# zkcrypto/bls12_381

Hardware: AMD Instinct MI355X
Metric: G1 MSM throughput (scalar-muls/sec) at 2^20 points (higher is better)
Workload: dtype u32 (14x28-bit limbs, 64-bit accumulators); 1 GPU; 2^20-point G1 MSM per MI355X, bases resident in HBM, scalars in HBM; one result per step; points_per_gpu=1048576, total_points=1048576, parallelism=shard1

## Files before the change

### bls12_381_amd/csrc/api_ctx.hip

```cpp
#define BLS_TU_NAME "api_ctx.hip"
#include "host.h"
#include "generators.hip.h"

__global__ void __launch_bounds__(256) k_fp_op(int op, const u32* __restrict__ a, const u32* __restrict__ b, u32* __restrict__ out, size_t n) {
  size_t i = (size_t)blockIdx.x * blockDim.x + threadIdx.x;
  if (i >= n) return;
  fe1 x = fe_from_ref(a + i * 12);
  fe1 y = b ? fe_from_ref(b + i * 12) : x;
  switch (op) {
    case 0: fe_to_ref(mul(x, y), out + i * 12); break;
    case 1: fe_to_ref(add(x, y), out + i * 12); break;
    case 2: fe_to_ref(sub(x, y), out + i * 12); break;
    case 3: fe_to_ref(sqr(x), out + i * 12); break;
    case 4: fe_to_ref(inv(x), out + i * 12); break;
    case 6: fe_to_ref(from_v16<2>(fe_inv_fermat_raw(to_v16(x))), out + i * 12); break;
    default: fe_to_ref(neg(x), out + i * 12); break;
  }
}
__global__ void __launch_bounds__(256) k_fp2_op(int op, const u32* __restrict__ a, const u32* __restrict__ b, u32* __restrict__ out, size_t n) {
  size_t i = (size_t)blockIdx.x * blockDim.x + threadIdx.x;
  if (i >= n) return;
  fe2_1 x = fe2_from_ref(a + i * 24);
  fe2_1 y = b ? fe2_from_ref(b + i * 24) : x;
  switch (op) {
// ... 145 lines not shown
  if (hipGetDeviceCount(&n) != hipSuccess || n <= 0) { g_err = "no HIP device"; return BLSGPU_ERR_NODEV; }
  if (device < 0 || device >= n) return bad("blsgpu_create: device index out of range");
  HIPCHK(hipSetDevice(device));
  blsgpu_ctx* c = new blsgpu_ctx();
  c->device = device;
  c->diag = diag_read(MMLP_MAX_K, ITEM_CAP_MAX, FR_COLS_LOG_MAX);
  if (c->diag.pairing_layout < 0) { delete c; return bad("blsgpu_create: BLSGPU_PAIRING_LAYOUT must be one of auto, pair, quad, wide"); }
  c->force_slow_sort = c->diag.force_slow_sort; c->no_glv = c->diag.no_glv; c->pairing_layout = c->diag.pairing_layout;
  c->mmlp_k = c->diag.mmlp_k; c->mml_impl = c->diag.mml_impl; c->h2c_split = c->diag.h2c_split; c->fr_cols_want = c->diag.fr_cols_want; c->item_cap = c->diag.item_cap;
  int rc = ctx_init(c);
  if (rc != BLSGPU_OK) { blsgpu_destroy(c); return rc; }
  *out = c;
  return BLSGPU_OK;
}
extern "C" void blsgpu_destroy(blsgpu_ctx* c) {
  if (!c) return;
  hipSetDevice(c->device);
  hipDeviceSynchronize();
  if (c->d_status) hipFree(c->d_status);
  if (c->d_wide) hipFree(c->d_wide);
  DevBuf* bufs[] = {&c->result, &c->io_a, &c->io_b, &c->io_c, &c->io_d, &c->io_e, &c->io_f, &c->io_out, &c->flags_a, &c->flags_b, &c->mml_vals, &c->fr_tw[0], &c->fr_tw[1], &c->fr_tmp, &c->fr_ninv, &c->fr_cs[0], &c->fr_cs[1], &c->fb_table[0], &c->fb_table[1], &c->fb_stage, &c->mmlp_work, &c->mmlp_out, &c->gt_one, &c->ver, &c->fold_c, &c->fold_d, &c->fold_result, &c->h2c_uniform, &c->seg_wsum, &c->seg_rec, &c->frs_agg[0], &c->frs_agg[1], &c->frs_carry[0], &c->frs_carry[1], &c->frs_lane};
  for (auto b : bufs) b->release();
  for (auto& sl : c->slot) {
    DevBuf* sb[] = {&sl.ent, &sl.sorted, &sl.hist, &sl.offs, &sl.cursor, &sl.bsum, &sl.items, &sl.heavy, &sl.ctrl, &sl.glv,
                    &sl.buckets, &sl.lvlR[0], &sl.lvlR[1], &sl.lvlT, &sl.tsum[0], &sl.tsum[1], &sl.wacc[0], &sl.wacc[1], &sl.wsums, &sl.result};
    for (auto b : sb) b->release();
    hipEvent_t evs[] = {sl.ev_in, sl.ev_front, sl.ev_acc, sl.ev_tail, sl.ev_k0, sl.ev_k1, sl.ev_tree};
    for (auto e : evs) if (e) hipEventDestroy(e);
    for (auto& e : sl.ev_lvl) if (e) hipEventDestroy(e);
    hipStream_t sts[] = {sl.front, sl.tail, sl.tail2};
    for (auto q : sts) if (q) hipStreamDestroy(q);
  }
  for (auto& e : c->ev) if (e) hipEventDestroy(e);
  for (auto& e : c->ev_fr) if (e) hipEventDestroy(e);
  for (auto& e : c->ev_fr_cs) if (e) hipEventDestroy(e);
  for (auto& e : c->ev_fb) if (e) hipEventDestroy(e);
  if (c->ev_gt_one) hipEventDestroy(c->ev_gt_one);
  if (c->fold_stream) hipStreamDestroy(c->fold_stream);
  if (c->pin_stage) hipHostFree(c->pin_stage);
  for (auto e : c->pin_ev) if (e) hipEventDestroy(e);
  if (c->ev_ver) hipEventDestroy(c->ev_ver);
  for (auto q : c->ver_stream) if (q) hipStreamDestroy(q);
  for (auto e : c->ev_ver_side) if (e) hipEventDestroy(e);
  if (c->ver_table) blsgpu_g2_prepared_free(c->ver_table);
  for (auto& e : c->bcache) if (e.b) blsgpu_bases_free(e.b);
  c->ktimer.destroy();
  if (c->acc_stream) hipStreamDestroy(c->acc_stream);
// ... 166 lines not shown
```

### bls12_381_amd/csrc/api_msm.hip

```cpp
#define BLS_TU_NAME "api_msm.hip"
#include "host.h"
#include "abi_kernels.hip.h"
#include "mulbatch.hip.h"
#include "msm_seg.hip.h"
#include "gntt.hip.h"

static void bases_drop(blsgpu_bases* b) {
  if (b->rec) hipFree(b->rec);
  if (b->endo) hipFree(b->endo);
  if (b->table) hipFree(b->table);
  if (b->ev_ready) hipEventDestroy(b->ev_ready);
  delete b;
}
static int bases_make_endo(blsgpu_ctx* c, blsgpu_bases* b, bool trusted) {
  if (!b->n) { b->subgroup = 1; return BLSGPU_OK; }
  if (b->group == 2 && b->n > ((size_t)1 << 22)) { b->subgroup = trusted ? 1 : (c->assume_subgroup ? 2 : 3); return BLSGPU_OK; }
  if (trusted) b->subgroup = 1;
  else if (c->assume_subgroup) b->subgroup = 2;
  else {
    u32 nbad = 0;
    HIPCHK(hipMemsetAsync(c->d_status + 1, 0, 4, c->stream));
    if (b->group == 1) KLAUNCH(k_bases_subgroup_check<FpPolicy>, dim3(nblk(b->n, 128)), dim3(128), 0, c->stream, b->rec, b->n, c->d_status + 1);
    else KLAUNCH(k_bases_subgroup_check<Fp2Policy>, dim3(nblk(b->n, 128)), dim3(128), 0, c->stream, b->rec, b->n, c->d_status + 1);
    LAUNCHCHK();
// ... 189 lines not shown
    KLAUNCH(k_proj_export<F>, dim3(1), dim3(256), 0, st, c->result.as<u32>(), (u32*)d_out_wire, (size_t)1);
    LAUNCHCHK();
    return BLSGPU_OK;
  }
  const bool merged = bases->table != nullptr;
  const bool glv = GroupTag<F>::id == 1 && !merged && bases->endo && !c->no_glv && !c->force_slow_sort && 2 * n <= ((size_t)1 << 24);
  const bool gls = GroupTag<F>::id == 2 && !merged && bases->endo && !c->no_glv && !c->force_slow_sort && 4 * n <= ((size_t)1 << 24);
  const size_t ns = glv ? 2 * n : gls ? 4 * n : n;
  const int sbits = glv ? 128 : gls ? 64 : 256;
  const int cw = merged ? bases->table_c : (c->msm_c ? c->msm_c : pick_window(ns, sbits));
  const int nwin = (sbits + cw - 1) / cw;
  const int nseg = merged ? 1 : nwin;
  const u32 nbw = 1u << (cw - 1);
  const size_t nb = (size_t)nseg * nbw;
  const size_t total = (size_t)nwin * ns;
  if (total > 0xfffffff0ull) return bad("msm: n * windows exceeds 2^32 entries");
  const bool fast_sort = merged || ((ns <= ((size_t)1 << 24)) && cw <= 16 && cw >= 2 && !c->force_slow_sort);
  const int key_bits = cw - 1;
  const int coarse_bits = merged ? (key_bits > 7 ? key_bits - 7 : 0) : (key_bits < 8 ? key_bits : 8);
  const int fine_bits = key_bits - coarse_bits;
  const int ncoarse = 1 << coarse_bits;
  const int nc = nseg * ncoarse;
  if (fast_sort && nc > SORT_MAX_COUNTERS) return bad("msm: window configuration exceeds the sort's counter table");
  if (!fast_sort && nblk(nb, 1024) > 4096) return bad("msm: too many buckets for the fallback sort (use a window <= 16)");
  int bad_alloc = 0;
  blsgpu_ctx::Slot& sl = c->slot[c->next_slot];
  c->next_slot = (c->next_slot + 1) % NSLOT;
  const bool single = !c->pipelining;
  hipStream_t ft = single ? st : sl.front, tt = single ? st : sl.tail;
  if (sl.tail_pending) { HIPCHK(hipStreamWaitEvent(ft, sl.ev_tail, 0)); HIPCHK(hipStreamWaitEvent(st, sl.ev_tail, 0)); }
  bad_alloc |= sl.ent.reserve(total * 4);
  bad_alloc |= sl.sorted.reserve(total * 4);
  {
    size_t hb = (nb > 3 * (size_t)SORT_MAX_COUNTERS + 4 ? nb : 3 * (size_t)SORT_MAX_COUNTERS + 4) * 4;
    bool fresh = sl.hist.cap < hb;
    bad_alloc |= sl.hist.reserve(hb);
    if (fresh && !bad_alloc) HIPCHK(hipMemsetAsync(sl.hist.p, 0, sl.hist.cap, ft));
  }
  if (!fast_sort) bad_alloc |= sl.cursor.reserve(total * 4);
  const int sform = c->scalar_form;
  const bool plain_mont = sform == SCALAR_MONT && !glv && !gls;
  if (glv) bad_alloc |= sl.glv.reserve(ns * 16);
  if (gls) bad_alloc |= sl.glv.reserve(ns * 8);
  if (plain_mont) bad_alloc |= sl.glv.reserve(n * 32);
  bad_alloc |= sl.offs.reserve((nb + 1) * 4);
  bad_alloc |= sl.bsum.reserve(4096 * 4);
  u32 cap = 128;
  while (cap < ITEM_CAP_MAX && (size_t)cap * nbw < 4 * ns) cap *= 2;
  if (c->item_cap) cap = c->item_cap;
  const size_t max_items = total / cap + nb + 1;
  const size_t max_records = nb + max_items;
  {
    blsgpu_ctx::Slot* g = &sl;
    bad_alloc |= g->items.reserve(max_items * sizeof(ItemDesc));
    bad_alloc |= g->heavy.reserve(2 * nb * sizeof(uint4));
    bad_alloc |= g->ctrl.reserve((4 + 2 * ITEM_BINS) * 4);
    size_t lvl = (nb / 2 + 1) * PW * 4;
    bool grow = g->buckets.cap < max_records * PW * 4 || g->lvlR[0].cap < lvl || g->lvlT.cap < 2 * lvl || g->wacc[0].cap < (size_t)nwin * 32 * PW * 4 || g->wsums.cap < (size_t)nwin * PW * 4;
    if (grow) { HIPCHK(hipStreamSynchronize(g->tail)); HIPCHK(hipStreamSynchronize(g->tail2)); HIPCHK(hipStreamSynchronize(st)); }
    bad_alloc |= g->buckets.reserve(max_records * PW * 4);
    bad_alloc |= g->lvlR[0].reserve(lvl); bad_alloc |= g->lvlR[1].reserve(lvl); bad_alloc |= g->lvlT.reserve(2 * lvl);
    bad_alloc |= g->tsum[0].reserve(lvl); bad_alloc |= g->tsum[1].reserve(lvl);
    bad_alloc |= g->wacc[0].reserve((size_t)nwin * 32 * PW * 4); bad_alloc |= g->wacc[1].reserve((size_t)nwin * 32 * PW * 4);
    bad_alloc |= g->wsums.reserve((size_t)nwin * PW * 4);
    bad_alloc |= g->result.reserve(PW * 4);
  }
  if (bad_alloc) { g_err = "hipMalloc(msm scratch) failed"; return BLSGPU_ERR_HIP; }
  const bool prof = c->profiling;
  auto mark = [&](int i) { if (prof) hipEventRecord(c->ev[i], ft); };
  if (ft != st) { HIPCHK(hipEventRecord(sl.ev_in, st)); HIPCHK(hipStreamWaitEvent(ft, sl.ev_in, 0)); }

  mark(0);
  if (plain_mont) {
    KLAUNCH(k_scalars_from_mont, dim3(nblk(n, 256)), dim3(256), 0, ft, (const u32*)d_scalars, sl.glv.as<u32>(), (int)n, c->status_word);
    LAUNCHCHK();
    d_scalars = sl.glv.p;
  }
  if (fast_sort) {
    u32* ghist = sl.hist.as<u32>();
    u32* gbase = ghist + SORT_MAX_COUNTERS;
    u32* gcur = gbase + SORT_MAX_COUNTERS + 1;
    if (sl.hist_dirty) { HIPCHK(hipMemsetAsync(ghist, 0, (size_t)SORT_MAX_COUNTERS * 4, ft)); sl.hist_dirty = false; }
    const unsigned tiles = nblk(ns, SORT_TILE);
    const u32* sort_in = (const u32*)d_scalars;
    if (glv) {
      KLAUNCH(k_glv_decompose, dim3(nblk(n, 256)), dim3(256), 0, ft, (const u32*)d_scalars, sl.glv.as<u32>(), (int)n, c->status_word, sform);
      sort_in = sl.glv.as<u32>();
      KLAUNCH(k_sort_hist<4>, dim3(tiles), dim3(SORT_THREADS), (size_t)nc * 4, ft, sort_in, ghist, (int)ns, cw, nwin, fine_bits, ncoarse, 0, c->status_word);
    } else if (gls) {
      KLAUNCH(k_gls_decompose, dim3(nblk(n, 256)), dim3(256), 0, ft, (const u32*)d_scalars, sl.glv.as<u32>(), (int)n, c->status_word, sform);
      sort_in = sl.glv.as<u32>();
      KLAUNCH(k_sort_hist<2>, dim3(tiles), dim3(SORT_THREADS), (size_t)nc * 4, ft, sort_in, ghist, (int)ns, cw, nwin, fine_bits, ncoarse, 0, c->status_word);
    } else {
      KLAUNCH(k_sort_hist<8>, dim3(tiles), dim3(SORT_THREADS), (size_t)nc * 4, ft, sort_in, ghist, (int)ns, cw, nwin, fine_bits, ncoarse, merged ? 1 : 0, c->status_word);
    }
    LAUNCHCHK();
    mark(1);
    KLAUNCH(k_sort_scan, dim3(1), dim3(1024), 0, ft, ghist, gbase, gcur, nc, sl.ctrl.as<u32>(), 4 + 2 * ITEM_BINS);
    LAUNCHCHK();
    mark(2);
    if (glv)
      KLAUNCH(k_sort_scatter<4>, dim3(tiles), dim3(SORT_THREADS), (size_t)nc * 8, ft, sort_in, gbase, gcur, sl.ent.as<u32>(), (int)ns, cw, nwin, fine_bits, ncoarse, 0, (u32)0);
    else if (gls)
      KLAUNCH(k_sort_scatter<2>, dim3(tiles), dim3(SORT_THREADS), (size_t)nc * 8, ft, sort_in, gbase, gcur, sl.ent.as<u32>(), (int)ns, cw, nwin, fine_bits, ncoarse, 0, (u32)0);
    else
      KLAUNCH(k_sort_scatter<8>, dim3(tiles), dim3(SORT_THREADS), (size_t)nc * 8, ft, sort_in, gbase, gcur, sl.ent.as<u32>(), (int)ns, cw, nwin,
                         fine_bits, ncoarse, merged ? 1 : 0, (u32)bases->n);
    KLAUNCH(k_sort_fine, dim3(nc), dim3(256), 0, ft, sl.ent.as<u32>(), gbase, sl.sorted.as<u32>(), sl.offs.as<u32>(), fine_bits, nc);
    LAUNCHCHK();
    mark(3);
  } else {
    sl.hist_dirty = true;
    HIPCHK(hipMemsetAsync(sl.hist.p, 0, nb * 4, ft));
    HIPCHK(hipMemsetAsync(sl.ctrl.p, 0, (4 + 2 * ITEM_BINS) * 4, ft));
    KLAUNCH(k_msm_digits, dim3(nblk(n, 256)), dim3(256), 0, ft, (const u32*)d_scalars, sl.ent.as<u32>(), sl.cursor.as<u32>(), sl.hist.as<u32>(), (int)n, cw, nwin, c->status_word);
    LAUNCHCHK();
    mark(1);
    unsigned sb = nblk(nb, 1024);
    KLAUNCH(k_scan_block_sums, dim3(sb), dim3(256), 0, ft, sl.hist.as<u32>(), sl.bsum.as<u32>(), (int)nb);
    KLAUNCH(k_scan_top, dim3(1), dim3(1024), 0, ft, sl.bsum.as<u32>(), (int)sb);
    KLAUNCH(k_scan_apply, dim3(sb), dim3(256), 0, ft, sl.hist.as<u32>(), sl.bsum.as<u32>(), sl.offs.as<u32>(), (int)nb);
    LAUNCHCHK();
    mark(2);
    KLAUNCH(k_msm_scatter, dim3(nblk(total, 256)), dim3(256), 0, ft, sl.ent.as<u32>(), sl.cursor.as<u32>(), sl.offs.as<u32>(), sl.sorted.as<u32>(),
                       (int)n, total);
    LAUNCHCHK();
    mark(3);
  }
  auto run_group = [&](blsgpu_ctx::Slot& gs, int g0, int ng, hipStream_t gft, hipStream_t gas, hipStream_t gtt, hipStream_t gt2, bool last) -> int {
  const size_t gnb = (size_t)ng * nbw;
  const size_t gmax_items = (size_t)(merged ? nwin : ng) * ns / cap + gnb + 1;
  const u32* goffs = sl.offs.as<u32>() + (size_t)g0 * nbw;
  u32* ctrl = gs.ctrl.as<u32>();
  u32* bins = ctrl + 4;
  u32* bcur = ctrl + 4 + ITEM_BINS;
// ... 555 lines not shown
```

### bls12_381_amd/csrc/host.h

```cpp
#pragma once
#include <hip/hip_runtime.h>
#include <stdint.h>
#include <stdio.h>
#include <string.h>
#include <string>
#include <cstdlib>
#include <vector>
#include <atomic>
#include <thread>
#include <array>
#include <mutex>
#include <condition_variable>
#include <functional>
#include <dlfcn.h>

#include "../../include/bls12_381_hip.h"
#include "convert.hip.h"
#include "scalar.hip.h"
#include "limits.h"
#include "diag.h"

using namespace bls;

inline thread_local std::string g_err;
// ... 78 lines not shown

#ifndef BLS_NSLOT
#define BLS_NSLOT 4
#endif
constexpr int NSLOT = BLS_NSLOT;
struct blsgpu_ctx {
  int device = 0;
  hipStream_t own_stream = nullptr, stream = nullptr;
  int msm_c = 0;
  bool profiling = false;
  bool pipelining = false;
  int acc_timing = 0;
  unsigned acc_tick = 0;
  double acc_ms_sum = 0.0; unsigned acc_count = 0;
  u32 item_cap = 0;
  int pairing_layout = 0;
  u32* d_wide = nullptr;
  size_t wide_off[4] = {0, 0, 0, 0};
  int wide_state = 0;
  std::string wide_why;
  int scalar_form = SCALAR_BYTES;
  bool assume_subgroup = false;
  bool no_glv = false;
  bool force_slow_sort = false;
  hipStream_t acc_stream = nullptr;
  hipEvent_t ev[9] = {};
  u32* d_status = nullptr;
  std::atomic<size_t> owner_thread{0};
  int owner_depth = 0;
  u32* status_word = nullptr;
  float phase_ms[8] = {0};
  struct Slot {
    hipStream_t front = nullptr, tail = nullptr, tail2 = nullptr;
    hipEvent_t ev_lvl[8] = {}, ev_tree = nullptr;
    hipEvent_t ev_in = nullptr, ev_front = nullptr, ev_acc = nullptr, ev_tail = nullptr;
    hipEvent_t ev_k0 = nullptr, ev_k1 = nullptr;
    bool k_pending = false;
    bool tail_pending = false;
    bool hist_dirty = false;
    unsigned long long seq = 0;
    DevBuf ent, sorted, hist, offs, cursor, bsum, items, heavy, ctrl, glv;
    DevBuf buckets, lvlR[2], lvlT, tsum[2], wacc[2], wsums, result;
  } slot[NSLOT];
  int next_slot = 0;
  unsigned long long msm_calls = 0;
  DevBuf result, io_a, io_b, io_c, io_d, io_e, io_f, io_out, flags_a, flags_b;
  DevBuf mml_vals;
  int mmlp_k = 0;
  int mml_impl = 0;
  struct BasesCacheEntry { int group; size_t n; uint64_t fp; blsgpu_bases* b; unsigned long long last; };
  std::vector<BasesCacheEntry> bcache;
  int bcache_cap = 0; unsigned long long bcache_tick = 0;
  bool bcache_verify = false;
  DevBuf mmlp_work, mmlp_out;
  DevBuf fold_c, fold_d, fold_result;
  bool on_fold_stream = false;
  hipStream_t fold_stream = nullptr;
  void* pin_stage = nullptr; hipEvent_t pin_ev[8] = {};
  bool pin_busy[8] = {};
  DevBuf gt_one; bool gt_one_ready = false; hipEvent_t ev_gt_one = nullptr;
  DevBuf ver;
  blsgpu_g2_prepared* ver_table = nullptr;
  bool ver_consts_ready = false; hipEvent_t ev_ver = nullptr;
  hipStream_t ver_stream[2] = {nullptr, nullptr}; hipEvent_t ev_ver_side[3] = {};
// ... 124 lines not shown
```

### bls12_381_amd/csrc/msm.hip.h

```cpp
#pragma once
#include <type_traits>
#include "convert.hip.h"
#include "scalar.hip.h"
#include "limits.h"
#include "team.hip.h"
#include "pairlane.hip.h"

namespace bls {

template <class F> struct Store;
template <> struct Store<FpPolicy> {
  static constexpr int AFF_WORDS = 32;
  static constexpr int PROJ_WORDS = 44;
  static constexpr int EL = NL;
  static DEV void ld(const u32* w, fe1& a) {
#pragma unroll
    for (int i = 0; i < NL; i++) a.l[i] = w[i];
  }
  template <class T> static DEV void st(u32* w, const T& a) {
#pragma unroll
    for (int i = 0; i < NL; i++) w[i] = a.l[i];
  }
  static DEV void ldw(const u32* w, fe& a) {
#pragma unroll
// ... 136 lines not shown
  load_aff<F>(rec + i * AW, q, inf);
  Proj<F> p; p.x = F::st(q.x); p.y = F::st(q.y); p.z = inf ? F::zero() : F::one();
  for (int w = 0; w < nwin; w++) {
    u32* r = table + ((size_t)w * n + i) * AW;
    if (w > 0) for (int k = 0; k < c; k++) p = pt_double<F>(p);
    bool zz = is_zero(p.z);
    auto zi = inv(p.z);
    auto x = canon_any(mul(p.x, zi));
    auto y = canon_any(mul(p.y, zi));
    Store<F>::st(r, x); Store<F>::st(r + EL, y);
    r[2 * EL] = zz ? 1 : 0;
    for (int j = 2 * EL + 1; j < AW; j++) r[j] = 0;
  }
}

#ifndef BLS_SORT_TILE
#define BLS_SORT_TILE 4096
#endif
#ifndef BLS_SORT_THREADS
#define BLS_SORT_THREADS 512
#endif
constexpr int SORT_TILE = BLS_SORT_TILE;
constexpr int SORT_THREADS = BLS_SORT_THREADS;
constexpr int SORT_MAX_COUNTERS = 8192;

template <int WORDS> struct DigitIter {
  u32 s[WORDS]; u32 carry, sign; int c; u32 nbw, mask;
  DEV void init(const u32* src, size_t i, int c_) {
    if constexpr (WORDS == 2) {
      uint2 a = *reinterpret_cast<const uint2*>(src + i * 2);
      s[0] = a.x; s[1] = a.y; sign = s[1] >> 31; s[1] &= 0x7fffffffu;
    } else {
      const uint4* sp = reinterpret_cast<const uint4*>(src + i * WORDS);
      uint4 a = sp[0];
      s[0] = a.x; s[1] = a.y; s[2] = a.z; s[3] = a.w;
      if constexpr (WORDS == 8) { uint4 b = sp[1]; s[4] = b.x; s[5] = b.y; s[6] = b.z; s[7] = b.w; sign = 0; }
      else { sign = s[3] >> 31; s[3] &= 0x7fffffffu; }
    }
    carry = 0; c = c_; nbw = 1u << (c - 1); mask = (1u << c) - 1;
  }
  DEV bool canonical() const { if constexpr (WORDS == 8) return scalar_is_canonical(s); else return true; }
  DEV void next(u32& mag, u32& neg) {
    u32 raw = (s[0] & mask) + carry;
#pragma unroll
    for (int j = 0; j < WORDS - 1; j++) s[j] = (s[j] >> c) | (s[j + 1] << (32 - c));
    s[WORDS - 1] >>= c;
    u32 over = raw > nbw;
// ... 138 lines not shown
  fe2_1 cx, cy;
  cx.c0 = fe1_const(zero); cx.c1 = fe1_const(px1); cy.c0 = fe1_const(py0); cy.c1 = fe1_const(py1);
  const u32* r = rec + i * AW;
  u32* o = out + 4 * i * AW;
  fe2_1 x, y; Store<Fp2Policy>::ld(r, x); Store<Fp2Policy>::ld(r + EL, y);
  const u32 flag = r[2 * EL];
  auto put = [&](int j, const fe2_1& px, const fe2_1& py) {
    u32* e = o + j * AW;
    Store<Fp2Policy>::st(e, px); Store<Fp2Policy>::st(e + EL, py);
    e[2 * EL] = flag;
    for (int t = 2 * EL + 1; t < AW; t++) e[t] = 0;
  };
  auto canon2 = [](const auto& v) { fe2_1 c; c.c0 = canon(v.c0); c.c1 = canon(v.c1); return c; };
  auto psi = [&](const fe2_1& px, const fe2_1& py, fe2_1& ox, fe2_1& oy) {
    ox = canon2(mul(conj(px), cx)); oy = canon2(mul(conj(py), cy));
  };
  put(0, x, y);
  fe2_1 x1, y1; psi(x, y, x1, y1); put(1, x1, y1);
  fe2_1 x2 = canon2(mul_fp(x, fe1_const(k2))), y2 = canon2(neg(y));
  put(2, x2, y2);
  fe2_1 x3, y3; psi(x2, y2, x3, y3); put(3, x3, y3);
}

template <int WORDS>
__global__ void __launch_bounds__(SORT_THREADS) k_sort_hist(const u32* __restrict__ scalars, u32* __restrict__ ghist, int n, int c, int nwin,
                                                   int fine_bits, int ncoarse, int merged, u32* __restrict__ status) {
  BLS_DYN_LDS(lh);
  const int nc = (merged ? 1 : nwin) * ncoarse;
  for (int i = threadIdx.x; i < nc; i += SORT_THREADS) lh[i] = 0;
  __syncthreads();
  for (int k = 0; k < SORT_TILE / SORT_THREADS; k++) {
    int i = blockIdx.x * SORT_TILE + k * SORT_THREADS + threadIdx.x;
    if (i < n) {
      DigitIter<WORDS> d; d.init(scalars, i, c);
      if (!d.canonical()) atomicOr(status, 1u);
      for (int w = 0; w < nwin; w++) {
        u32 mag, neg; d.next(mag, neg);
        if (mag) atomicAdd(&lh[(merged ? 0 : w) * ncoarse + ((mag - 1) >> fine_bits)], 1u);
      }
    }
  }
  __syncthreads();
  for (int i = threadIdx.x; i < nc; i += SORT_THREADS) if (lh[i]) atomicAdd(&ghist[i], lh[i]);
}
__global__ void __launch_bounds__(1024) k_sort_scan(u32* __restrict__ ghist, u32* __restrict__ gbase, u32* __restrict__ gcur, int nc,
                                                    u32* __restrict__ ctrl, int nctrl) {
  __shared__ u32 sh[SORT_MAX_COUNTERS];
  __shared__ u32 part[1024];
  const int per = (nc + 1023) / 1024;
  u32 t = 0;
  for (int j = 0; j < per; j++) { int i = threadIdx.x * per + j; u32 v = i < nc ? ghist[i] : 0; if (i < nc) sh[i] = v; t += v; }
  part[threadIdx.x] = t;
  __syncthreads();
  for (int st = 1; st < 1024; st <<= 1) {
    u32 x = (int)threadIdx.x >= st ? part[threadIdx.x - st] : 0;
    __syncthreads();
    part[threadIdx.x] += x;
    __syncthreads();
  }
  u32 run = part[threadIdx.x] - t;
  for (int j = 0; j < per; j++) { int i = threadIdx.x * per + j; if (i < nc) { gbase[i] = run; gcur[i] = 0; ghist[i] = 0; run += sh[i]; } }
  if (threadIdx.x == 1023) gbase[nc] = part[1023];
  for (int i = threadIdx.x; i < nctrl; i += 1024) ctrl[i] = 0;
}
template <int WORDS>
__global__ void __launch_bounds__(SORT_THREADS) k_sort_scatter(const u32* __restrict__ scalars, const u32* __restrict__ gbase, u32* __restrict__ gcur,
                                                      u32* __restrict__ coarse_out, int n, int c, int nwin, int fine_bits, int ncoarse,
                                                      int merged, u32 stride) {
  BLS_DYN_LDS(lh);
  const int nc = (merged ? 1 : nwin) * ncoarse;
  u32* lbase = lh + nc;
  for (int i = threadIdx.x; i < nc; i += SORT_THREADS) lh[i] = 0;
  __syncthreads();
  for (int k = 0; k < SORT_TILE / SORT_THREADS; k++) {
    int i = blockIdx.x * SORT_TILE + k * SORT_THREADS + threadIdx.x;
    if (i < n) {
      DigitIter<WORDS> d; d.init(scalars, i, c);
      for (int w = 0; w < nwin; w++) {
        u32 mag, neg; d.next(mag, neg);
        if (mag) atomicAdd(&lh[(merged ? 0 : w) * ncoarse + ((mag - 1) >> fine_bits)], 1u);
      }
    }
  }
  __syncthreads();
  for (int i = threadIdx.x; i < nc; i += SORT_THREADS) {
    u32 cnt = lh[i];
    lbase[i] = cnt ? gbase[i] + atomicAdd(&gcur[i], cnt) : 0;
    lh[i] = 0;
  }
  __syncthreads();
  const u32 fmask = (1u << fine_bits) - 1;
  for (int k = 0; k < SORT_TILE / SORT_THREADS; k++) {
    int i = blockIdx.x * SORT_TILE + k * SORT_THREADS + threadIdx.x;
    if (i < n) {
      DigitIter<WORDS> d; d.init(scalars, i, c);
      for (int w = 0; w < nwin; w++) {
        u32 mag, neg; d.next(mag, neg);
        if (mag) {
          int ci = (merged ? 0 : w) * ncoarse + ((mag - 1) >> fine_bits);
          u32 r = atomicAdd(&lh[ci], 1u);
          u32 idx = merged ? (u32)w * stride + (u32)i : (u32)i;
          coarse_out[lbase[ci] + r] = (idx << 8) | (neg << 7) | ((mag - 1) & fmask);
        }
      }
    }
  }
}
__global__ void __launch_bounds__(256) k_sort_fine(const u32* __restrict__ coarse_in, const u32* __restrict__ gbase, u32* __restrict__ sorted,
                                                   u32* __restrict__ offs, int fine_bits, int nc) {
  __shared__ u32 cnt[128];
  __shared__ u32 base[128];
  const int region = blockIdx.x;
  const u32 beg = gbase[region], end = gbase[region + 1];
  const int nfine = 1 << fine_bits;
  if (threadIdx.x < 128) cnt[threadIdx.x] = 0;
  __syncthreads();
  for (u32 j = beg + threadIdx.x; j < end; j += 256) atomicAdd(&cnt[coarse_in[j] & 127u], 1u);
  __syncthreads();
  if (threadIdx.x == 0) {
    u32 run = beg;
    for (int f = 0; f < nfine; f++) { base[f] = run; run += cnt[f]; }
  }
  __syncthreads();
  if ((int)threadIdx.x < nfine) { offs[(size_t)region * nfine + threadIdx.x] = base[threadIdx.x]; cnt[threadIdx.x] = 0; }
  if (region == nc - 1 && threadIdx.x == 0) offs[(size_t)nc * nfine] = end;
  __syncthreads();
  for (u32 j = beg + threadIdx.x; j < end; j += 256) {
    u32 e = coarse_in[j];
    u32 f = e & 127u;
    u32 r = atomicAdd(&cnt[f], 1u);
    sorted[base[f] + r] = (e >> 8) | ((e & 0x80u) << 24);
  }
}

__global__ void __launch_bounds__(256) k_scan_block_sums(const u32* __restrict__ in, u32* __restrict__ bsum, int n) {
  __shared__ u32 sh[256];
  int base = blockIdx.x * 1024;
  u32 t = 0;
  for (int j = 0; j < 4; j++) {
    int idx = base + threadIdx.x * 4 + j;
    if (idx < n) t += in[idx];
  }
  sh[threadIdx.x] = t;
  __syncthreads();
  for (int s = 128; s > 0; s >>= 1) {
    if ((int)threadIdx.x < s) sh[threadIdx.x] += sh[threadIdx.x + s];
    __syncthreads();
  }
  if (threadIdx.x == 0) bsum[blockIdx.x] = sh[0];
}
__global__ void __launch_bounds__(1024) k_scan_top(u32* __restrict__ bsum, int nb) {
  __shared__ u32 sh[4096];
  for (int i = threadIdx.x; i < 4096; i += 1024) sh[i] = i < nb ? bsum[i] : 0;
  __syncthreads();
// ... 538 lines not shown
```

Baseline: 382.3 million scalar-muls/s.

## Replace atomic global sort scatter with per-slice count table and LDS-staged coalesced writes

The MSM bucket sort now writes per-slice coarse counts into a table, row-scans it, and gives each block deterministic output offsets instead of global atomics on a cursor. The scatter stages entries in LDS, sized to the device's maximum, and writes them out in contiguous runs found by binary search. An ordered variant keeps stable order per wave for small coarse counts. The fine sort now loads uint4 vectors and stages in LDS with per-wave counters. This targets scattered uncoalesced global writes and atomic contention, at the cost of large LDS use, lower occupancy and an extra kernel launch.

```diff
diff --git a/bls12_381_amd/csrc/api_ctx.hip b/bls12_381_amd/csrc/api_ctx.hip
--- a/bls12_381_amd/csrc/api_ctx.hip
+++ b/bls12_381_amd/csrc/api_ctx.hip
@@ -191,7 +191,7 @@
   DevBuf* bufs[] = {&c->result, &c->io_a, &c->io_b, &c->io_c, &c->io_d, &c->io_e, &c->io_f, &c->io_out, &c->flags_a, &c->flags_b, &c->mml_vals, &c->fr_tw[0], &c->fr_tw[1], &c->fr_tmp, &c->fr_ninv, &c->fr_cs[0], &c->fr_cs[1], &c->fb_table[0], &c->fb_table[1], &c->fb_stage, &c->mmlp_work, &c->mmlp_out, &c->gt_one, &c->ver, &c->fold_c, &c->fold_d, &c->fold_result, &c->h2c_uniform, &c->seg_wsum, &c->seg_rec, &c->frs_agg[0], &c->frs_agg[1], &c->frs_carry[0], &c->frs_carry[1], &c->frs_lane};
   for (auto b : bufs) b->release();
   for (auto& sl : c->slot) {
-    DevBuf* sb[] = {&sl.ent, &sl.sorted, &sl.hist, &sl.offs, &sl.cursor, &sl.bsum, &sl.items, &sl.heavy, &sl.ctrl, &sl.glv,
+    DevBuf* sb[] = {&sl.ent, &sl.sorted, &sl.hist, &sl.tcnt, &sl.offs, &sl.cursor, &sl.bsum, &sl.items, &sl.heavy, &sl.ctrl, &sl.glv,
                     &sl.buckets, &sl.lvlR[0], &sl.lvlR[1], &sl.lvlT, &sl.tsum[0], &sl.tsum[1], &sl.wacc[0], &sl.wacc[1], &sl.wsums, &sl.result};
     for (auto b : sb) b->release();
     hipEvent_t evs[] = {sl.ev_in, sl.ev_front, sl.ev_acc, sl.ev_tail, sl.ev_k0, sl.ev_k1, sl.ev_tree};
diff --git a/bls12_381_amd/csrc/api_msm.hip b/bls12_381_amd/csrc/api_msm.hip
--- a/bls12_381_amd/csrc/api_msm.hip
+++ b/bls12_381_amd/csrc/api_msm.hip
@@ -235,6 +235,19 @@
   const int ncoarse = 1 << coarse_bits;
   const int nc = nseg * ncoarse;
   if (fast_sort && nc > SORT_MAX_COUNTERS) return bad("msm: window configuration exceeds the sort's counter table");
+  int sort_tile = SORT_TILE, sort_span = 1; unsigned sort_slices = 1; size_t scatter_lds = 0;
+  const bool sort_ordered = ncoarse <= SORT_ORDERED_COARSE;
+  const long sort_fixed = sort_ordered ? 10240 : 1024;
+  const long sort_arrays = (sort_ordered ? 2 : 3) * (long)nc + 1;
+  if (fast_sort) {
+    if (c->lds_max < 0) { int v = 0; c->lds_max = hipDeviceGetAttribute(&v, hipDeviceAttributeMaxSharedMemoryPerBlock, c->device) == hipSuccess ? v : 65536; }
+    const long stage_words = ((long)c->lds_max - sort_fixed) / 4 - sort_arrays;
+    while (sort_tile > 1 && (long)sort_tile * nwin > stage_words) sort_tile >>= 1;
+    if ((long)sort_tile * nwin > stage_words) return bad("msm: window configuration exceeds the sort's LDS");
+    while ((size_t)nc * nblk(ns, (size_t)sort_tile * sort_span) > SORT_TABLE_MAX) sort_span *= 2;
+    sort_slices = nblk(ns, (size_t)sort_tile * sort_span);
+    scatter_lds = ((size_t)sort_arrays + (size_t)sort_tile * nwin) * 4;
+  }
   if (!fast_sort && nblk(nb, 1024) > 4096) return bad("msm: too many buckets for the fallback sort (use a window <= 16)");
   int bad_alloc = 0;
   blsgpu_ctx::Slot& sl = c->slot[c->next_slot];
@@ -242,14 +255,10 @@
   const bool single = !c->pipelining;
   hipStream_t ft = single ? st : sl.front, tt = single ? st : sl.tail;
   if (sl.tail_pending) { HIPCHK(hipStreamWaitEvent(ft, sl.ev_tail, 0)); HIPCHK(hipStreamWaitEvent(st, sl.ev_tail, 0)); }
-  bad_alloc |= sl.ent.reserve(total * 4);
+  bad_alloc |= sl.ent.reserve(total * 4 + 16);
   bad_alloc |= sl.sorted.reserve(total * 4);
-  {
-    size_t hb = (nb > 3 * (size_t)SORT_MAX_COUNTERS + 4 ? nb : 3 * (size_t)SORT_MAX_COUNTERS + 4) * 4;
-    bool fresh = sl.hist.cap < hb;
-    bad_alloc |= sl.hist.reserve(hb);
-    if (fresh && !bad_alloc) HIPCHK(hipMemsetAsync(sl.hist.p, 0, sl.hist.cap, ft));
-  }
+  bad_alloc |= sl.hist.reserve((nb > 2 * (size_t)SORT_MAX_COUNTERS + 4 ? nb : 2 * (size_t)SORT_MAX_COUNTERS + 4) * 4);
+  if (fast_sort) bad_alloc |= sl.tcnt.reserve((size_t)nc * sort_slices * 4);
   if (!fast_sort) bad_alloc |= sl.cursor.reserve(total * 4);
   const int sform = c->scalar_form;
   const bool plain_mont = sform == SCALAR_MONT && !glv && !gls;
@@ -292,38 +301,47 @@
   if (fast_sort) {
     u32* ghist = sl.hist.as<u32>();
     u32* gbase = ghist + SORT_MAX_COUNTERS;
-    u32* gcur = gbase + SORT_MAX_COUNTERS + 1;
-    if (sl.hist_dirty) { HIPCHK(hipMemsetAsync(ghist, 0, (size_t)SORT_MAX_COUNTERS * 4, ft)); sl.hist_dirty = false; }
-    const unsigned tiles = nblk(ns, SORT_TILE);
+    u32* table = sl.tcnt.as<u32>();
+    const int per_slice = sort_tile * sort_span;
+    const int mrg = merged ? 1 : 0;
+    const u32 stride = merged ? (u32)bases->n : 0;
     const u32* sort_in = (const u32*)d_scalars;
     if (glv) {
       KLAUNCH(k_glv_decompose, dim3(nblk(n, 256)), dim3(256), 0, ft, (const u32*)d_scalars, sl.glv.as<u32>(), (int)n, c->status_word, sform);
       sort_in = sl.glv.as<u32>();
-      KLAUNCH(k_sort_hist<4>, dim3(tiles), dim3(SORT_THREADS), (size_t)nc * 4, ft, sort_in, ghist, (int)ns, cw, nwin, fine_bits, ncoarse, 0, c->status_word);
+      KLAUNCH(k_sort_count<4>, dim3(sort_slices), dim3(SORT_THREADS), (size_t)nc * 4, ft, sort_in, table, (int)ns, cw, nwin, fine_bits, ncoarse, 0, c->status_word, per_slice);
     } else if (gls) {
       KLAUNCH(k_gls_decompose, dim3(nblk(n, 256)), dim3(256), 0, ft, (const u32*)d_scalars, sl.glv.as<u32>(), (int)n, c->status_word, sform);
       sort_in = sl.glv.as<u32>();
-      KLAUNCH(k_sort_hist<2>, dim3(tiles), dim3(SORT_THREADS), (size_t)nc * 4, ft, sort_in, ghist, (int)ns, cw, nwin, fine_bits, ncoarse, 0, c->status_word);
+      KLAUNCH(k_sort_count<2>, dim3(sort_slices), dim3(SORT_THREADS), (size_t)nc * 4, ft, sort_in, table, (int)ns, cw, nwin, fine_bits, ncoarse, 0, c->status_word, per_slice);
     } else {
-      KLAUNCH(k_sort_hist<8>, dim3(tiles), dim3(SORT_THREADS), (size_t)nc * 4, ft, sort_in, ghist, (int)ns, cw, nwin, fine_bits, ncoarse, merged ? 1 : 0, c->status_word);
+      KLAUNCH(k_sort_count<8>, dim3(sort_slices), dim3(SORT_THREADS), (size_t)nc * 4, ft, sort_in, table, (int)ns, cw, nwin, fine_bits, ncoarse, mrg, c->status_word, per_slice);
     }
     LAUNCHCHK();
     mark(1);
-    KLAUNCH(k_sort_scan, dim3(1), dim3(1024), 0, ft, ghist, gbase, gcur, nc, sl.ctrl.as<u32>(), 4 + 2 * ITEM_BINS);
+    KLAUNCH(k_sort_rows, dim3(nc), dim3(256), 0, ft, table, ghist, (int)sort_slices);
+    KLAUNCH(k_sort_scan, dim3(1), dim3(1024), 0, ft, (const u32*)ghist, gbase, nc, sl.ctrl.as<u32>(), 4 + 2 * ITEM_BINS);
     LAUNCHCHK();
     mark(2);
-    if (glv)
-      KLAUNCH(k_sort_scatter<4>, dim3(tiles), dim3(SORT_THREADS), (size_t)nc * 8, ft, sort_in, gbase, gcur, sl.ent.as<u32>(), (int)ns, cw, nwin, fine_bits, ncoarse, 0, (u32)0);
-    else if (gls)
-      KLAUNCH(k_sort_scatter<2>, dim3(tiles), dim3(SORT_THREADS), (size_t)nc * 8, ft, sort_in, gbase, gcur, sl.ent.as<u32>(), (int)ns, cw, nwin, fine_bits, ncoarse, 0, (u32)0);
-    else
-      KLAUNCH(k_sort_scatter<8>, dim3(tiles), dim3(SORT_THREADS), (size_t)nc * 8, ft, sort_in, gbase, gcur, sl.ent.as<u32>(), (int)ns, cw, nwin,
-                         fine_bits, ncoarse, merged ? 1 : 0, (u32)bases->n);
-    KLAUNCH(k_sort_fine, dim3(nc), dim3(256), 0, ft, sl.ent.as<u32>(), gbase, sl.sorted.as<u32>(), sl.offs.as<u32>(), fine_bits, nc);
+    if (!c->scatter_lds_set) {
+      const int most = c->lds_max - 1024, most_o = c->lds_max - 10240;
+      HIPCHK(hipFuncSetAttribute((const void*)k_sort_scatter<4>, hipFuncAttributeMaxDynamicSharedMemorySize, most));
+      HIPCHK(hipFuncSetAttribute((const void*)k_sort_scatter<2>, hipFuncAttributeMaxDynamicSharedMemorySize, most));
+      HIPCHK(hipFuncSetAttribute((const void*)k_sort_scatter<8>, hipFuncAttributeMaxDynamicSharedMemorySize, most));
+      HIPCHK(hipFuncSetAttribute((const void*)k_sort_scatter_ordered<4>, hipFuncAttributeMaxDynamicSharedMemorySize, most_o));
+      HIPCHK(hipFuncSetAttribute((const void*)k_sort_scatter_ordered<2>, hipFuncAttributeMaxDynamicSharedMemorySize, most_o));
+      HIPCHK(hipFuncSetAttribute((const void*)k_sort_scatter_ordered<8>, hipFuncAttributeMaxDynamicSharedMemorySize, most_o));
+      c->scatter_lds_set = true;
+    }
+#define SORT_SCATTER(W) do { \
+      if (sort_ordered) KLAUNCH(k_sort_scatter_ordered<W>, dim3(sort_slices), dim3(SORT_ORDERED_THREADS), scatter_lds, ft, sort_in, (const u32*)gbase, (const u32*)table, sl.ent.as<u32>(), (int)ns, cw, nwin, fine_bits, ncoarse, mrg, stride, sort_tile, sort_span); \
+      else KLAUNCH(k_sort_scatter<W>, dim3(sort_slices), dim3(SORT_SCATTER_THREADS), scatter_lds, ft, sort_in, (const u32*)gbase, (const u32*)table, sl.ent.as<u32>(), (int)ns, cw, nwin, fine_bits, ncoarse, mrg, stride, sort_tile, sort_span); } while (0)
+    if (glv) SORT_SCATTER(4); else if (gls) SORT_SCATTER(2); else SORT_SCATTER(8);
+#undef SORT_SCATTER
+    KLAUNCH(k_sort_fine, dim3(nc), dim3(256), 0, ft, sl.ent.as<u32>(), (const u32*)gbase, sl.sorted.as<u32>(), sl.offs.as<u32>(), fine_bits, nc);
     LAUNCHCHK();
     mark(3);
   } else {
-    sl.hist_dirty = true;
     HIPCHK(hipMemsetAsync(sl.hist.p, 0, nb * 4, ft));
     HIPCHK(hipMemsetAsync(sl.ctrl.p, 0, (4 + 2 * ITEM_BINS) * 4, ft));
     KLAUNCH(k_msm_digits, dim3(nblk(n, 256)), dim3(256), 0, ft, (const u32*)d_scalars, sl.ent.as<u32>(), sl.cursor.as<u32>(), sl.hist.as<u32>(), (int)n, cw, nwin, c->status_word);
diff --git a/bls12_381_amd/csrc/host.h b/bls12_381_amd/csrc/host.h
--- a/bls12_381_amd/csrc/host.h
+++ b/bls12_381_amd/csrc/host.h
@@ -124,6 +124,8 @@
   int scalar_form = SCALAR_BYTES;
   bool assume_subgroup = false;
   bool no_glv = false;
+  int lds_max = -1;
+  bool scatter_lds_set = false;
   bool force_slow_sort = false;
   hipStream_t acc_stream = nullptr;
   hipEvent_t ev[9] = {};
@@ -139,9 +141,8 @@
     hipEvent_t ev_k0 = nullptr, ev_k1 = nullptr;
     bool k_pending = false;
     bool tail_pending = false;
-    bool hist_dirty = false;
     unsigned long long seq = 0;
-    DevBuf ent, sorted, hist, offs, cursor, bsum, items, heavy, ctrl, glv;
+    DevBuf ent, sorted, hist, tcnt, offs, cursor, bsum, items, heavy, ctrl, glv;
     DevBuf buckets, lvlR[2], lvlT, tsum[2], wacc[2], wsums, result;
   } slot[NSLOT];
   int next_slot = 0;
diff --git a/bls12_381_amd/csrc/msm.hip.h b/bls12_381_amd/csrc/msm.hip.h
--- a/bls12_381_amd/csrc/msm.hip.h
+++ b/bls12_381_amd/csrc/msm.hip.h
@@ -182,7 +182,10 @@
 #endif
 constexpr int SORT_TILE = BLS_SORT_TILE;
 constexpr int SORT_THREADS = BLS_SORT_THREADS;
+constexpr int SORT_SCATTER_THREADS = 1024;
 constexpr int SORT_MAX_COUNTERS = 8192;
+constexpr size_t SORT_TABLE_MAX = (size_t)1 << 22;
+constexpr int SORT_FINE_CAP = 12288;
 
 template <int WORDS> struct DigitIter {
   u32 s[WORDS]; u32 carry, sign; int c; u32 nbw, mask;
@@ -367,114 +370,295 @@
   fe2_1 x3, y3; psi(x2, y2, x3, y3); put(3, x3, y3);
 }
 
+DEV u32 wave_incl_scan(u32 v) {
+  const unsigned lane = threadIdx.x & 63u;
+  for (unsigned d = 1; d < 64; d <<= 1) { u32 t = (u32)__shfl_up((int)v, d, 64); if (lane >= d) v += t; }
+  return v;
+}
+DEV void block_excl_scan(const u32* src, u32* dst, int n, u32* ws) {
+  const int nt = (int)blockDim.x, per = (n + nt - 1) / nt, lane = threadIdx.x & 63, wave = threadIdx.x >> 6;
+  u32 t = 0;
+  for (int j = 0; j < per; j++) { int i = (int)threadIdx.x * per + j; if (i < n) t += src[i]; }
+  const u32 incl = wave_incl_scan(t);
+  if (lane == 63) ws[wave] = incl;
+  __syncthreads();
+  if (wave == 0) { u32 w = lane < (nt >> 6) ? ws[lane] : 0; u32 wi = wave_incl_scan(w); ws[lane] = wi - w; }
+  __syncthreads();
+  u32 run = ws[wave] + incl - t;
+  for (int j = 0; j < per; j++) { int i = (int)threadIdx.x * per + j; if (i < n) { u32 v = src[i]; dst[i] = run; run += v; } }
+  if ((int)threadIdx.x == nt - 1) dst[n] = run;
+  __syncthreads();
+}
+
+template <int T>
+DEV void sort_stage_out(const u32* lofs, const u32* dst, const u32* stage, u32* __restrict__ coarse_out, int nc) {
+  constexpr int U = 8;
+  const u32 total = lofs[nc];
+  int top = 1;
+  while (top * 2 < nc) top *= 2;
+  for (u32 j0 = threadIdx.x; j0 < total; j0 += U * T) {
+    int pos[U];
+#pragma unroll
+    for (int u = 0; u < U; u++) pos[u] = 0;
+    for (int h = top; h > 0; h >>= 1) {
+#pragma unroll
+      for (int u = 0; u < U; u++) {
+        const int m = pos[u] + h < nc ? pos[u] + h : nc;
+        pos[u] = lofs[m] <= j0 + (u32)(u * T) ? m : pos[u];
+      }
+    }
+#pragma unroll
+    for (int u = 0; u < U; u++) {
+      const u32 j = j0 + (u32)(u * T);
+      if (j < total) coarse_out[dst[pos[u]] + j] = stage[j];
+    }
+  }
+}
+
 template <int WORDS>
-__global__ void __launch_bounds__(SORT_THREADS) k_sort_hist(const u32* __restrict__ scalars, u32* __restrict__ ghist, int n, int c, int nwin,
-                                                   int fine_bits, int ncoarse, int merged, u32* __restrict__ status) {
+__global__ void __launch_bounds__(SORT_THREADS) k_sort_count(const u32* __restrict__ scalars, u32* __restrict__ table, int n, int c, int nwin,
+                                                    int fine_bits, int ncoarse, int merged, u32* __restrict__ status, int per_block) {
   BLS_DYN_LDS(lh);
   const int nc = (merged ? 1 : nwin) * ncoarse;
   for (int i = threadIdx.x; i < nc; i += SORT_THREADS) lh[i] = 0;
   __syncthreads();
-  for (int k = 0; k < SORT_TILE / SORT_THREADS; k++) {
-    int i = blockIdx.x * SORT_TILE + k * SORT_THREADS + threadIdx.x;
-    if (i < n) {
-      DigitIter<WORDS> d; d.init(scalars, i, c);
-      if (!d.canonical()) atomicOr(status, 1u);
-      for (int w = 0; w < nwin; w++) {
-        u32 mag, neg; d.next(mag, neg);
-        if (mag) atomicAdd(&lh[(merged ? 0 : w) * ncoarse + ((mag - 1) >> fine_bits)], 1u);
-      }
-    }
-  }
-  __syncthreads();
-  for (int i = threadIdx.x; i < nc; i += SORT_THREADS) if (lh[i]) atomicAdd(&ghist[i], lh[i]);
-}
-__global__ void __launch_bounds__(1024) k_sort_scan(u32* __restrict__ ghist, u32* __restrict__ gbase, u32* __restrict__ gcur, int nc,
-                                                    u32* __restrict__ ctrl, int nctrl) {
-  __shared__ u32 sh[SORT_MAX_COUNTERS];
-  __shared__ u32 part[1024];
-  const int per = (nc + 1023) / 1024;
-  u32 t = 0;
-  for (int j = 0; j < per; j++) { int i = threadIdx.x * per + j; u32 v = i < nc ? ghist[i] : 0; if (i < nc) sh[i] = v; t += v; }
-  part[threadIdx.x] = t;
-  __syncthreads();
-  for (int st = 1; st < 1024; st <<= 1) {
-    u32 x = (int)threadIdx.x >= st ? part[threadIdx.x - st] : 0;
-    __syncthreads();
-    part[threadIdx.x] += x;
-    __syncthreads();
-  }
-  u32 run = part[threadIdx.x] - t;
-  for (int j = 0; j < per; j++) { int i = threadIdx.x * per + j; if (i < nc) { gbase[i] = run; gcur[i] = 0; ghist[i] = 0; run += sh[i]; } }
-  if (threadIdx.x == 1023) gbase[nc] = part[1023];
+  const int lo = blockIdx.x * per_block, hi = n - lo < per_block ? n : lo + per_block;
+  for (int i = lo + threadIdx.x; i < hi; i += SORT_THREADS) {
+    DigitIter<WORDS> d; d.init(scalars, i, c);
+    if (!d.canonical()) atomicOr(status, 1u);
+    for (int w = 0; w < nwin; w++) {
+      u32 mag, neg; d.next(mag, neg);
+      if (mag) atomicAdd(&lh[(merged ? 0 : w) * ncoarse + ((mag - 1) >> fine_bits)], 1u);
+    }
+  }
+  __syncthreads();
+  for (int i = threadIdx.x; i < nc; i += SORT_THREADS) table[(size_t)i * gridDim.x + blockIdx.x] = lh[i];
+}
+__global__ void __launch_bounds__(256) k_sort_rows(u32* __restrict__ table, u32* __restrict__ ghist, int B) {
+  __shared__ u32 ws[4];
+  u32* row = table + (size_t)blockIdx.x * B;
+  const int lane = threadIdx.x & 63, wave = threadIdx.x >> 6;
+  u32 carry = 0;
+  for (int base = 0; base < B; base += 1024) {
+    u32 v[4], t = 0;
+    for (int j = 0; j < 4; j++) { int i = base + (int)threadIdx.x * 4 + j; v[j] = i < B ? row[i] : 0; t += v[j]; }
+    const u32 incl = wave_incl_scan(t);
+    if (lane == 63) ws[wave] = incl;
+    __syncthreads();
+    u32 below = 0, all = 0;
+    for (int w = 0; w < 4; w++) { u32 x = ws[w]; if (w < wave) below += x; all += x; }
+    u32 run = carry + below + incl - t;
+    for (int j = 0; j < 4; j++) { int i = base + (int)threadIdx.x * 4 + j; if (i < B) row[i] = run; run += v[j]; }
+    carry += all;
+    __syncthreads();
+  }
+  if (threadIdx.x == 0) ghist[blockIdx.x] = carry;
+}
+__global__ void __launch_bounds__(1024) k_sort_scan(const u32* __restrict__ ghist, u32* __restrict__ gbase, int nc, u32* __restrict__ ctrl, int nctrl) {
+  __shared__ u32 sh[SORT_MAX_COUNTERS + 1];
+  __shared__ u32 ws[64];
+  for (int i = threadIdx.x; i < nc; i += 1024) sh[i] = ghist[i];
+  __syncthreads();
+  block_excl_scan(sh, sh, nc, ws);
+  for (int i = threadIdx.x; i <= nc; i += 1024) gbase[i] = sh[i];
   for (int i = threadIdx.x; i < nctrl; i += 1024) ctrl[i] = 0;
 }
 template <int WORDS>
-__global__ void __launch_bounds__(SORT_THREADS) k_sort_scatter(const u32* __restrict__ scalars, const u32* __restrict__ gbase, u32* __restrict__ gcur,
+__global__ void __launch_bounds__(SORT_SCATTER_THREADS) k_sort_scatter(const u32* __restrict__ scalars, const u32* __restrict__ gbase, const u32* __restrict__ table,
                                                       u32* __restrict__ coarse_out, int n, int c, int nwin, int fine_bits, int ncoarse,
-                                                      int merged, u32 stride) {
-  BLS_DYN_LDS(lh);
+                                                      int merged, u32 stride, int tile, int span) {
+  BLS_DYN_LDS(lds);
+  __shared__ u32 ws[64];
+  constexpr int T = SORT_SCATTER_THREADS;
   const int nc = (merged ? 1 : nwin) * ncoarse;
-  u32* lbase = lh + nc;
-  for (int i = threadIdx.x; i < nc; i += SORT_THREADS) lh[i] = 0;
-  __syncthreads();
-  for (int k = 0; k < SORT_TILE / SORT_THREADS; k++) {
-    int i = blockIdx.x * SORT_TILE + k * SORT_THREADS + threadIdx.x;
-    if (i < n) {
+  u32* cnt = lds;
+  u32* lofs = cnt + nc;
+  u32* dst = lofs + nc + 1;
+  u32* stage = dst + nc;
+  for (int i = threadIdx.x; i < nc; i += T) { dst[i] = gbase[i] + table[(size_t)i * gridDim.x + blockIdx.x]; cnt[i] = 0; }
+  __syncthreads();
+  const u32 fmask = (1u << fine_bits) - 1;
+  for (int s = 0; s < span; s++) {
+    const int lo = (blockIdx.x * span + s) * tile;
+    if (lo >= n) break;
+    const int hi = n - lo < tile ? n : lo + tile;
+    for (int i = lo + threadIdx.x; i < hi; i += T) {
       DigitIter<WORDS> d; d.init(scalars, i, c);
       for (int w = 0; w < nwin; w++) {
         u32 mag, neg; d.next(mag, neg);
-        if (mag) atomicAdd(&lh[(merged ? 0 : w) * ncoarse + ((mag - 1) >> fine_bits)], 1u);
+        if (mag) atomicAdd(&cnt[(merged ? 0 : w) * ncoarse + ((mag - 1) >> fine_bits)], 1u);
       }
     }
-  }
-  __syncthreads();
-  for (int i = threadIdx.x; i < nc; i += SORT_THREADS) {
-    u32 cnt = lh[i];
-    lbase[i] = cnt ? gbase[i] + atomicAdd(&gcur[i], cnt) : 0;
-    lh[i] = 0;
-  }
-  __syncthreads();
-  const u32 fmask = (1u << fine_bits) - 1;
-  for (int k = 0; k < SORT_TILE / SORT_THREADS; k++) {
-    int i = blockIdx.x * SORT_TILE + k * SORT_THREADS + threadIdx.x;
-    if (i < n) {
+    __syncthreads();
+    block_excl_scan(cnt, lofs, nc, ws);
+    for (int i = threadIdx.x; i < nc; i += T) { dst[i] -= lofs[i]; cnt[i] = 0; }
+    __syncthreads();
+    for (int i = lo + threadIdx.x; i < hi; i += T) {
       DigitIter<WORDS> d; d.init(scalars, i, c);
       for (int w = 0; w < nwin; w++) {
         u32 mag, neg; d.next(mag, neg);
         if (mag) {
-          int ci = (merged ? 0 : w) * ncoarse + ((mag - 1) >> fine_bits);
-          u32 r = atomicAdd(&lh[ci], 1u);
-          u32 idx = merged ? (u32)w * stride + (u32)i : (u32)i;
-          coarse_out[lbase[ci] + r] = (idx << 8) | (neg << 7) | ((mag - 1) & fmask);
+          const int ci = (merged ? 0 : w) * ncoarse + ((mag - 1) >> fine_bits);
+          const u32 r = atomicAdd(&cnt[ci], 1u);
+          const u32 idx = merged ? (u32)w * stride + (u32)i : (u32)i;
+          stage[lofs[ci] + r] = (idx << 8) | (neg << 7) | ((mag - 1) & fmask);
         }
       }
     }
+    __syncthreads();
+    sort_stage_out<T>(lofs, dst, stage, coarse_out, nc);
+    __syncthreads();
+    for (int i = threadIdx.x; i < nc; i += T) { dst[i] += lofs[i + 1]; cnt[i] = 0; }
+    __syncthreads();
+  }
+}
+constexpr int SORT_ORDERED_THREADS = 512;
+constexpr int SORT_ORDERED_WAVES = SORT_ORDERED_THREADS / 64;
+constexpr int SORT_ORDERED_COARSE = 256;
+template <int WORDS>
+__global__ void __launch_bounds__(SORT_ORDERED_THREADS) k_sort_scatter_ordered(const u32* __restrict__ scalars, const u32* __restrict__ gbase, const u32* __restrict__ table,
+                                                      u32* __restrict__ coarse_out, int n, int c, int nwin, int fine_bits, int ncoarse,
+                                                      int merged, u32 stride, int tile, int span) {
+  BLS_DYN_LDS(lds);
+  __shared__ u32 ws[64];
+  __shared__ u32 wtab[SORT_ORDERED_WAVES][SORT_ORDERED_COARSE];
+  __shared__ u32 wfill[SORT_ORDERED_COARSE];
+  constexpr int T = SORT_ORDERED_THREADS, K = SORT_TILE / T;
+  const int nc = (merged ? 1 : nwin) * ncoarse;
+  u32* lofs = lds;
+  u32* dst = lofs + nc + 1;
+  u32* stage = dst + nc;
+  u32* mine = wtab[threadIdx.x >> 6];
+  for (int i = threadIdx.x; i < nc; i += T) { dst[i] = gbase[i] + table[(size_t)i * gridDim.x + blockIdx.x]; lofs[i] = 0; }
+  __syncthreads();
+  const u32 fmask = (1u << fine_bits) - 1;
+  for (int s = 0; s < span; s++) {
+    const int lo = (blockIdx.x * span + s) * tile;
+    if (lo >= n) break;
+    const int hi = n - lo < tile ? n : lo + tile;
+    DigitIter<WORDS> d[K];
+#pragma unroll
+    for (int k = 0; k < K; k++) {
+      const int i = lo + k * T + (int)threadIdx.x;
+      if (i < hi) {
+        d[k].init(scalars, i, c);
+        for (int w = 0; w < nwin; w++) {
+          u32 mag, neg; d[k].next(mag, neg);
+          if (mag) atomicAdd(&lofs[(merged ? 0 : w) * ncoarse + ((mag - 1) >> fine_bits)], 1u);
+        }
+        d[k].init(scalars, i, c);
+      }
+    }
+    if ((int)threadIdx.x < ncoarse) wfill[threadIdx.x] = 0;
+    __syncthreads();
+    block_excl_scan(lofs, lofs, nc, ws);
+    for (int i = threadIdx.x; i < nc; i += T) dst[i] -= lofs[i];
+    for (int w = 0; w < nwin; w++) {
+      for (int i = threadIdx.x; i < SORT_ORDERED_WAVES * SORT_ORDERED_COARSE; i += T) (&wtab[0][0])[i] = 0;
+      __syncthreads();
+      u32 r[K], e[K], co[K];
+#pragma unroll
+      for (int k = 0; k < K; k++) {
+        const int i = lo + k * T + (int)threadIdx.x;
+        r[k] = 0xffffffffu; e[k] = 0; co[k] = 0;
+        if (i < hi) {
+          u32 mag, neg; d[k].next(mag, neg);
+          if (mag) {
+            co[k] = (mag - 1) >> fine_bits;
+            const u32 idx = merged ? (u32)w * stride + (u32)i : (u32)i;
+            e[k] = (idx << 8) | (neg << 7) | ((mag - 1) & fmask);
+            r[k] = atomicAdd(&mine[co[k]], 1u);
+          }
+        }
+      }
+      __syncthreads();
+      if ((int)threadIdx.x < ncoarse) {
+        u32 run = merged ? wfill[threadIdx.x] : 0;
+        for (int v = 0; v < SORT_ORDERED_WAVES; v++) { const u32 x = wtab[v][threadIdx.x]; wtab[v][threadIdx.x] = run; run += x; }
+        if (merged) wfill[threadIdx.x] = run;
+      }
+      __syncthreads();
+      const int cb = merged ? 0 : w * ncoarse;
+#pragma unroll
+      for (int k = 0; k < K; k++)
+        if (r[k] != 0xffffffffu) stage[lofs[cb + (int)co[k]] + mine[co[k]] + r[k]] = e[k];
+      __syncthreads();
+    }
+    sort_stage_out<T>(lofs, dst, stage, coarse_out, nc);
+    __syncthreads();
+    for (int i = threadIdx.x; i < nc; i += T) dst[i] += lofs[i + 1];
+    __syncthreads();
+    for (int i = threadIdx.x; i < nc; i += T) lofs[i] = 0;
+    __syncthreads();
   }
 }
 __global__ void __launch_bounds__(256) k_sort_fine(const u32* __restrict__ coarse_in, const u32* __restrict__ gbase, u32* __restrict__ sorted,
                                                    u32* __restrict__ offs, int fine_bits, int nc) {
-  __shared__ u32 cnt[128];
-  __shared__ u32 base[128];
+  __shared__ u32 wcnt[4][128];
+  __shared__ u32 wofs[4][128];
+  __shared__ u32 stage[SORT_FINE_CAP];
+  constexpr int NV = (SORT_FINE_CAP / 4 + 1 + 255) / 256;
   const int region = blockIdx.x;
   const u32 beg = gbase[region], end = gbase[region + 1];
   const int nfine = 1 << fine_bits;
-  if (threadIdx.x < 128) cnt[threadIdx.x] = 0;
-  __syncthreads();
-  for (u32 j = beg + threadIdx.x; j < end; j += 256) atomicAdd(&cnt[coarse_in[j] & 127u], 1u);
-  __syncthreads();
-  if (threadIdx.x == 0) {
-    u32 run = beg;
-    for (int f = 0; f < nfine; f++) { base[f] = run; run += cnt[f]; }
-  }
-  __syncthreads();
-  if ((int)threadIdx.x < nfine) { offs[(size_t)region * nfine + threadIdx.x] = base[threadIdx.x]; cnt[threadIdx.x] = 0; }
+  const bool fits = end - beg <= (u32)SORT_FINE_CAP;
+  const u32 a0 = beg & ~3u;
+  u32* mine = wcnt[threadIdx.x >> 6];
+  const u32* myofs = wofs[threadIdx.x >> 6];
+  uint4 v[NV];
+  for (int i = threadIdx.x; i < 512; i += 256) (&wcnt[0][0])[i] = 0;
+  __syncthreads();
+  if (fits) {
+#pragma unroll
+    for (int k = 0; k < NV; k++) {
+      const u32 p = a0 + (u32)(k * 256 + (int)threadIdx.x) * 4;
+      if (p < end) {
+        v[k] = *reinterpret_cast<const uint4*>(coarse_in + p);
+        if (p >= beg) atomicAdd(&mine[v[k].x & 127u], 1u);
+        if (p + 1 >= beg && p + 1 < end) atomicAdd(&mine[v[k].y & 127u], 1u);
+        if (p + 2 >= beg && p + 2 < end) atomicAdd(&mine[v[k].z & 127u], 1u);
+        if (p + 3 >= beg && p + 3 < end) atomicAdd(&mine[v[k].w & 127u], 1u);
+      }
+    }
+  } else {
+    for (u32 j = beg + threadIdx.x; j < end; j += 256) atomicAdd(&mine[coarse_in[j] & 127u], 1u);
+  }
+  __syncthreads();
+  if (threadIdx.x < 64) {
+    u32 c[2][4], t = 0;
+    for (int h = 0; h < 2; h++) for (int w = 0; w < 4; w++) { c[h][w] = wcnt[w][2 * threadIdx.x + h]; t += c[h][w]; }
+    u32 run = wave_incl_scan(t) - t;
+    for (int h = 0; h < 2; h++) {
+      const int f = 2 * threadIdx.x + h;
+      if (f < nfine) offs[(size_t)region * nfine + f] = beg + run;
+      for (int w = 0; w < 4; w++) { wofs[w][f] = run; run += c[h][w]; }
+    }
+  }
   if (region == nc - 1 && threadIdx.x == 0) offs[(size_t)nc * nfine] = end;
   __syncthreads();
-  for (u32 j = beg + threadIdx.x; j < end; j += 256) {
-    u32 e = coarse_in[j];
-    u32 f = e & 127u;
-    u32 r = atomicAdd(&cnt[f], 1u);
-    sorted[base[f] + r] = (e >> 8) | ((e & 0x80u) << 24);
+  for (int i = threadIdx.x; i < 512; i += 256) (&wcnt[0][0])[i] = 0;
+  __syncthreads();
+  if (fits) {
+    auto place = [&](u32 e) { const u32 f = e & 127u; const u32 r = atomicAdd(&mine[f], 1u); stage[myofs[f] + r] = (e >> 8) | ((e & 0x80u) << 24); };
+#pragma unroll
+    for (int k = 0; k < NV; k++) {
+      const u32 p = a0 + (u32)(k * 256 + (int)threadIdx.x) * 4;
+      if (p < end) {
+        if (p >= beg) place(v[k].x);
+        if (p + 1 >= beg && p + 1 < end) place(v[k].y);
+        if (p + 2 >= beg && p + 2 < end) place(v[k].z);
+        if (p + 3 >= beg && p + 3 < end) place(v[k].w);
+      }
+    }
+    __syncthreads();
+    for (u32 j = threadIdx.x; j < end - beg; j += 256) sorted[beg + j] = stage[j];
+  } else {
+    for (u32 j = beg + threadIdx.x; j < end; j += 256) {
+      u32 e = coarse_in[j];
+      u32 f = e & 127u;
+      u32 r = atomicAdd(&mine[f], 1u);
+      sorted[beg + myofs[f] + r] = (e >> 8) | ((e & 0x80u) << 24);
+    }
   }
 }
 
```

New measurement: 381.8 million scalar-muls/s. Within noise of the previous version (-0.1%).
